# VirtualPlants/tissue_analysis

Measured on AMD Instinct MI355X. Metric: Mvoxels/s full-feature extraction, 1024^3 vol/50k labels; % HBM roofline, higher is better.
Workload: dtype u64; 1 GPU; C4: 1024x1024x1024 uint32, 50000 seeds (21839 labels present), features=0x1f, Z-slab x1; voxels_per_gpu=1073741824, label_dtype=uint32, steps_in_flight=1, per_label_reduce=all

## Files before the change

tissue_analysis_amd/csrc/kernels_basic.hip:

```cpp
#include "ta_kernels.h"

namespace ta {

__global__ void __launch_bounds__(256) init_kernel(uint64_t* sums, int32_t* boxes, uint64_t nlabels,
                                                   uint32_t* flags, uint32_t* cursor, uint64_t* hot_rows) {
    const uint64_t tid = (uint64_t)blockIdx.x * blockDim.x + threadIdx.x;
    const uint64_t nthreads = (uint64_t)gridDim.x * blockDim.x;
    const uint64_t nsum2 = nlabels * NSUM / 2;
    ulonglong2* s2 = reinterpret_cast<ulonglong2*>(sums);
    for (uint64_t i = tid; i < nsum2; i += nthreads) s2[i] = make_ulonglong2(0ull, 0ull);
    const uint64_t nbox2 = nlabels * NBOX / 2;
    int2* b2 = reinterpret_cast<int2*>(boxes);
    for (uint64_t i = tid; i < nbox2; i += nthreads) b2[i] = make_int2(INT32_MAX, INT32_MAX);
    if (tid < NFLAGS) flags[tid] = 0u;
    if (tid == 0) {
        *cursor = 0u;
        *reinterpret_cast<uint64_t**>(flags + HOT_PTR_WORD) = hot_rows;
    }
}

void launch_init_accumulators(hipStream_t s, uint64_t* sums, int32_t* boxes, uint64_t nlabels,
                              uint32_t* flags, uint32_t* pair_cursor, uint64_t* hot_rows) {
    uint64_t work = nlabels * NSUM / 2;
    int blocks = (int)((work + 255) / 256);
// ... 99 lines not shown
        }
    }
    for (uint64_t i = nvec * VEC + tid; i < nvox; i += nthreads) m = max(m, (uint32_t)vol[i]);
#pragma unroll
    for (int off = 32; off > 0; off >>= 1) m = max(m, (uint32_t)__shfl_xor((int)m, off, 64));
    if ((threadIdx.x & 63) == 0) atomicMax(out, m);
}

void launch_max_label(hipStream_t s, const void* vol, int itemsize, uint64_t nvox, uint32_t* out_dev) {
    (void)hipMemsetAsync(out_dev, 0, sizeof(uint32_t), s);
    if (nvox == 0) return;
    uint64_t blocks = (nvox / (16 / itemsize) + 255) / 256;
    if (blocks < 1) blocks = 1;
    if (blocks > 2048) blocks = 2048;
    if (itemsize == 2)
        hipLaunchKernelGGL(max_label_kernel<uint16_t>, dim3((unsigned)blocks), dim3(256), 0, s,
                           (const uint16_t*)vol, nvox, out_dev);
    else
        hipLaunchKernelGGL(max_label_kernel<uint32_t>, dim3((unsigned)blocks), dim3(256), 0, s,
                           (const uint32_t*)vol, nvox, out_dev);
}

constexpr int COLLECT_PER_THREAD = 8;
__device__ __forceinline__ void publish_small(const uint32_t* small, uint32_t* publish, int nwords, int tid) {
    if (tid < nwords) {
        const uint32_t v = __hip_atomic_load(&small[tid], __ATOMIC_RELAXED, __HIP_MEMORY_SCOPE_AGENT);
        __hip_atomic_store(&publish[tid], v, __ATOMIC_RELAXED, __HIP_MEMORY_SCOPE_SYSTEM);
    }
}

__device__ __forceinline__ void pairs_collect_block(const PairTable& pt, uint64_t* out_keys, uint64_t* out_faces,
                                                    uint32_t* cursor, const uint32_t block) {
    __shared__ uint32_t wave_tot[4];
    __shared__ uint32_t block_base;
    const uint64_t cap = (uint64_t)pt.mask + 1;
    const int tid = threadIdx.x, lane = tid & 63, w = tid >> 6;
    const uint64_t lo = (uint64_t)block * (256 * COLLECT_PER_THREAD);
    uint64_t k[COLLECT_PER_THREAD];
    uint32_t mine = 0;
#pragma unroll
    for (int i = 0; i < COLLECT_PER_THREAD; ++i) {
        const uint64_t h = lo + (uint64_t)i * 256 + tid;
        k[i] = h < cap ? pt.keys[h] : EMPTY_KEY;
    }
#pragma unroll
    for (int i = 0; i < COLLECT_PER_THREAD; ++i) mine += k[i] != EMPTY_KEY;
    uint32_t incl = mine;
#pragma unroll
    for (int off = 1; off < 64; off <<= 1) {
        const uint32_t up = (uint32_t)__shfl_up((int)incl, off, 64);
        if (lane >= off) incl += up;
    }
    if (lane == 63) wave_tot[w] = incl;
    __syncthreads();
    if (tid == 0) {
        const uint32_t total = wave_tot[0] + wave_tot[1] + wave_tot[2] + wave_tot[3];
        block_base = total ? atomicAdd(cursor, total) : 0u;
    }
    __syncthreads();
    uint32_t pos = block_base + incl - mine;
    for (int i = 0; i < w; ++i) pos += wave_tot[i];
#pragma unroll
    for (int i = 0; i < COLLECT_PER_THREAD; ++i) {
        if (k[i] == EMPTY_KEY) continue;
        const uint64_t h = lo + (uint64_t)i * 256 + tid;
        out_keys[pos] = k[i];
        out_faces[3ull * pos + 0] = pt.faces[3 * h + 0];
        out_faces[3ull * pos + 1] = pt.faces[3 * h + 1];
        out_faces[3ull * pos + 2] = pt.faces[3 * h + 2];
        ++pos;
        pt.keys[h] = EMPTY_KEY;
        pt.faces[3 * h + 0] = 0; pt.faces[3 * h + 1] = 0; pt.faces[3 * h + 2] = 0;
    }
}

__global__ void __launch_bounds__(256) pairs_collect_kernel(PairTable pt, uint64_t* out_keys,
                                                            uint64_t* out_faces, uint32_t* cursor) {
    pairs_collect_block(pt, out_keys, out_faces, cursor, blockIdx.x);
}

void launch_pairs_collect(hipStream_t s, const PairTable& pt, uint64_t* out_keys, uint64_t* out_faces,
                          uint32_t* cursor) {
    const uint64_t cap = (uint64_t)pt.mask + 1;
    const uint64_t per_block = 256 * COLLECT_PER_THREAD;
    const uint64_t blocks = (cap + per_block - 1) / per_block;
    hipLaunchKernelGGL(pairs_collect_kernel, dim3((unsigned)blocks), dim3(256), 0, s, pt, out_keys,
                       out_faces, cursor);
}

__global__ void __launch_bounds__(256) pairs_insert_kernel(PairTable pt, const uint64_t* keys,
                                                           const uint64_t* faces, uint64_t n,
                                                           uint32_t* flags) {
    for (uint64_t i = (uint64_t)blockIdx.x * blockDim.x + threadIdx.x; i < n;
         i += (uint64_t)gridDim.x * blockDim.x) {
        const uint64_t k = keys[i];
// ... 108 lines not shown
        }
        if (i >= n) continue;
        const uint64_t k = blk[XHDR + i];
        if (k == EMPTY_KEY) continue;
        const uint64_t* f = blk + XHDR + cap + 3 * i;
        pair_add_global(pt, (uint32_t)(k >> 32), (uint32_t)k, f[0], f[1], f[2], flags);
    }
}

void launch_pairs_insert_blocks(hipStream_t s, const PairTable& pt, const uint64_t* blocks, int nblocks,
                                uint64_t cap, uint32_t* flags) {
    const uint64_t total = (uint64_t)nblocks * cap;
    if (total == 0) return;
    uint64_t grid = (total + 255) / 256;
    if (grid > 4096) grid = 4096;
    hipLaunchKernelGGL(pairs_insert_blocks_kernel, dim3((unsigned)grid), dim3(256), 0, s, pt, blocks, nblocks,
                       cap, flags);
}

__global__ void __launch_bounds__(256) pairs_clear_kernel(PairTable pt) {
    const uint64_t cap = (uint64_t)pt.mask + 1;
    for (uint64_t h = (uint64_t)blockIdx.x * blockDim.x + threadIdx.x; h < cap;
         h += (uint64_t)gridDim.x * blockDim.x) {
        pt.keys[h] = EMPTY_KEY;
        pt.faces[3 * h + 0] = 0; pt.faces[3 * h + 1] = 0; pt.faces[3 * h + 2] = 0;
    }
}

void launch_pairs_clear(hipStream_t s, const PairTable& pt) {
    uint64_t cap = (uint64_t)pt.mask + 1;
    uint64_t blocks = (cap + 255) / 256;
    if (blocks > 2048) blocks = 2048;
    hipLaunchKernelGGL(pairs_clear_kernel, dim3((unsigned)blocks), dim3(256), 0, s, pt);
}

struct HotFold {
    const uint64_t* rows; uint32_t nrows;
    const void* vol; int itemsize; int64_t corner;
    uint64_t* sums; int32_t* boxes; uint32_t max_label;
};

__device__ __forceinline__ void hot_reduce_block(const HotFold& H, const uint32_t block, const uint32_t nblocks) {
    __shared__ uint64_t part[256];
    const uint32_t hot = H.itemsize == 2 ? (uint32_t)((const uint16_t*)H.vol)[H.corner] : ((const uint32_t*)H.vol)[H.corner];
    if (hot > H.max_label) return;
    const int col = threadIdx.x & (HOTW - 1), lanegrp = threadIdx.x / HOTW;
    const bool is_sum = col < NSUM;
    int64_t acc = is_sum ? 0 : (int64_t)INT32_MAX;
// ... 394 lines not shown
```

tissue_analysis_amd/csrc/kernels_scan.hip:

```cpp
#include "ta_sweep_common.h"

#include <type_traits>

#include <hip/hip_ext.h>

namespace ta {

constexpr int FCAP = TA_FCAP, RCAP = TA_RCAP;
constexpr uint32_t ROWID_MASK = 0x7FFFFC00u;
constexpr uint32_t ROW_END = 0x80000000u;
constexpr uint32_t NO_ROW = 0xFFFFFFFFu;

typedef __attribute__((address_space(3))) uint32_t* lds_u32;

template <bool ADJ>
struct __attribute__((aligned(16))) ScanWaveLds {
    uint2 frec[ADJ ? FCAP + 1 : 1];
    uint32_t cql[RCAP + 2], cqc[RCAP + 2];
};

template <int NW, bool ADJ, typename PACK>
struct __attribute__((aligned(16))) ScanLds {
    using Pack = PACK;
    ScanWaveLds<ADJ> wave[WAVES];
// ... 124 lines not shown
        k = S.lkeys[h];
    }
    if (slot >= 0) {
        unsigned long long* row = (unsigned long long*)&S.lsum[slot * NW];
        uint64_t w[4];
        LDS::Pack::template pack<MOM2>(L, w);
#ifndef TA_ABL_NOSUMS
#pragma unroll
        for (int k = 0; k < NW; ++k) atomicAdd(row + k, (unsigned long long)w[k]);
#endif
        uint32_t* box = &S.lbox[slot * 8];
        const uint4 cur = *reinterpret_cast<const uint4*>(box);
        const uint2 cur2 = *reinterpret_cast<const uint2*>(box + 4);
#ifdef TA_ABL_NOBOX
        const bool grows = (mna + cur.x + cur2.x == 0x12345u);
#else
        const bool grows = (mna < cur.x) | (mnb < cur.y) | (mnc < cur.z) | (mxa > cur.w) | (mxb > cur2.x) | (mxc > cur2.y);
#endif
        if (grows) {
            atomicMin(box + 0, mna); atomicMin(box + 1, mnb); atomicMin(box + 2, mnc);
            atomicMax(box + 3, mxa); atomicMax(box + 4, mxb); atomicMax(box + 5, mxc);
        }
    } else {
        const SweepArgs* A = cold_args(kp);
        LocalSums Lc;
        Lc.n = L.n; Lc.sa = L.sa; Lc.sb = L.sb; Lc.sc = L.sc; Lc.saa = L.saa; Lc.sab = L.sab;
        Lc.sac = L.sac; Lc.sbb = L.sbb; Lc.sbc = L.sbc; Lc.scc = L.scc;
        uint32_t bx[6];
        bx[0] = mna; bx[1] = mnb; bx[2] = mnc; bx[3] = mxa; bx[4] = mxb; bx[5] = mxc;
        label_spill_global(A->sums, A->boxes, A->flags, A->max_label, label, &Lc, S.frame[0], S.frame[1], S.frame[2], bx);
    }
}

__device__ __forceinline__ uint32_t scan_pair_hash(uint32_t lo, uint32_t hi) {
    const uint32_t h = mad24_const(hi, 0x85EBCBu, mul24_const(lo, 0x9E3779u));
    return (h >> (24 - PSLOTS_LOG2)) & (PSLOTS - 1);
}

template <typename LDS>
__device__ __forceinline__ void scan_pair_add(const SweepArgs* kp, LDS& S, uint32_t lo, uint32_t hi, uint32_t axis, uint32_t h,
                                              uint64_t k) {
    const uint64_t key = ((uint64_t)lo << 32) | hi;
    int slot = -1;
#pragma nounroll
    for (int probe = 0; probe < PPROBE; ++probe) {
        if (k == EMPTY_KEY) {
            k = atomicCAS((unsigned long long*)&S.pkeys[h], (unsigned long long)EMPTY_KEY, (unsigned long long)key);
            if (k == EMPTY_KEY) k = key;
        }
        if (k == key) { slot = (int)h; break; }
        h = (h + 1) & (PSLOTS - 1);
        k = S.pkeys[h];
    }
// ... 256 lines not shown
#ifdef TA_ABL_SHARE1
        unsigned long long* row = (unsigned long long*)&S.lsum[((lslot + (uint32_t)lane) & (LSLOTS - 1)) * NW];
#else
        unsigned long long* row = (unsigned long long*)&S.lsum[lslot * NW];
#endif
        uint64_t w[4];
        LDS::Pack::template pack<MOM2>(L, w);
#pragma unroll
        for (int k = 0; k < NW; ++k) atomicAdd(row + k, (unsigned long long)w[k]);
#ifdef TA_ABL_NOBOXHOT
        const bool grows = false;
#else
        const bool grows = (al < cur.x) | (bl < cur.y) | (c0 < cur.z) | (al > cur.w) | (bl > cur2.x) | (kk - 1u > cur2.y);
#endif
        if (grows) {
            uint32_t* box = &S.lbox[lslot * 8];
            atomicMin(box + 0, al); atomicMin(box + 1, bl); atomicMin(box + 2, c0);
            atomicMax(box + 3, al); atomicMax(box + 4, bl); atomicMax(box + 5, kk - 1u);
        }
    }
    if (spill) {
        if (ppend) { const SweepArgs* A = cold_args(kp); pair_spill_global(A->pairs, A->flags, plo, phi, 2u, 1u); }
        if (lpend) {
            const SweepArgs* A = cold_args(kp);
            LocalSums Lc;
            Lc.n = L.n; Lc.sa = L.sa; Lc.sb = L.sb; Lc.sc = L.sc; Lc.saa = L.saa; Lc.sab = L.sab;
            Lc.sac = L.sac; Lc.sbb = L.sbb; Lc.sbc = L.sbc; Lc.scc = L.scc;
            uint32_t bx[6];
            bx[0] = al; bx[1] = bl; bx[2] = c0; bx[3] = al; bx[4] = bl; bx[5] = kk - 1u;
            label_spill_global(A->sums, A->boxes, A->flags, A->max_label, label, &Lc, S.frame[0], S.frame[1], S.frame[2], bx);
        }
    }
    rcount = rem;
    __builtin_amdgcn_fence(__ATOMIC_ACQ_REL, "wavefront");
}

template <typename T, int VPL>
__device__ __forceinline__ void scan_load_strip(const T* row_c0, bool row_ok, uint32_t lane_off, int64_t c, int64_t n2,
                                                uint32_t (&dst)[VPL], bool& bad) {
    const T* lane_p = reinterpret_cast<const T*>(reinterpret_cast<const char*>(row_c0) + lane_off);
#pragma unroll
    for (int j = 0; j < VPL; ++j) {
        const bool ok = row_ok && c + j < n2;
        dst[j] = ok ? (uint32_t)lane_p[j] : INVALID_LABEL;
        if (sizeof(T) == 4) bad |= ok && dst[j] == INVALID_LABEL;
    }
}

typedef uint32_t u32x4 __attribute__((ext_vector_type(4)));

#define SCAN_VARIANTS(X)                                                             \
    X(scan_kernel,           ROWS_HALO, 104)         \
    X(scan_pad_kernel,       ROWS_HALO, 120)              \
// ... 645 lines not shown
```

tissue_analysis_amd/csrc/ta_api.hip:

```cpp
#include "ta_ctx.h"

#include <cstdarg>
#include <cstdio>
#include <cstdlib>
#include <new>

static thread_local std::string g_err;

int fail(int code, const char* fmt, ...) {
    char buf[512];
    va_list ap;
    va_start(ap, fmt);
    vsnprintf(buf, sizeof(buf), fmt, ap);
    va_end(ap);
    g_err = buf;
    return code;
}

namespace {

int ensure_pair_table(ta_ctx* c, int log2cap) {
    if (c->pair_log2 == log2cap && c->pkeys.p) return TA_OK;
    const uint64_t cap = 1ull << log2cap;
    int rc;
    if ((rc = c->pkeys.reserve(cap * 8)) != TA_OK) return rc;
    if ((rc = c->pfaces.reserve(cap * 24)) != TA_OK) return rc;
    if ((rc = c->out_keys.reserve(cap * 8)) != TA_OK) return rc;
    if ((rc = c->out_faces.reserve(cap * 24)) != TA_OK) return rc;
    c->pair_log2 = log2cap;
    c->table_clean = false;
    return TA_OK;
}

int auto_pair_log2(uint32_t max_label) {
    uint64_t want = 16ull * ((uint64_t)max_label + 1);
    int l = 16;
    while ((1ull << l) < want && l < 28) ++l;
    return l;
}

double sampled_event_density(ta_ctx* c) {
    const int64_t owned = c->mdims[0] - c->first_owned;
    if (owned <= 0 || c->mdims[1] <= 0 || c->mdims[2] <= 0 || !c->vol) return -1.0;
    const int nsample = (int)std::min<int64_t>(8, owned);
    DevBuf d;
    if (d.reserve((uint64_t)nsample * sizeof(uint64_t)) != TA_OK) return -1.0;
    const size_t plane_bytes = (size_t)c->mdims[1] * c->mdims[2] * c->itemsize;
    for (int k = 0; k < nsample; ++k) {
        const int64_t p = c->first_owned + ((2 * k + 1) * owned) / (2 * nsample);
// ... 310 lines not shown
    if (e == hipSuccess && rc == TA_OK) e = hipHostMalloc((void**)&c->h_small, SMALL_WORDS * sizeof(uint32_t), hipHostMallocMapped);
    if (e == hipSuccess && rc == TA_OK) {
        void* dp = nullptr;
        if (hipHostGetDevicePointer(&dp, c->h_small, 0) == hipSuccess) c->h_small_dev = (uint32_t*)dp;
        else (void)hipGetLastError();
    }
    if (e != hipSuccess || rc != TA_OK) {
        if (e != hipSuccess) rc = fail(e == hipErrorOutOfMemory ? TA_ENOMEM : TA_EHIP, "ta_ctx_create: %s", hipGetErrorString(e));
        const std::string keep = g_err;
        (void)ta_ctx_destroy(c);
        g_err = keep;
        return rc;
    }
    memset(c->h_small, 0, SMALL_WORDS * sizeof(uint32_t));
    *out = c;
    return TA_OK;
}

TA_API int ta_ctx_destroy(ta_ctx* c) {
    if (!c) return TA_OK;
    (void)hipSetDevice(c->device);
    if (c->stream) (void)hipStreamSynchronize(c->stream);
    c->owned_vol.release(); c->own_sums.release(); c->own_boxes.release();
    c->pkeys.release(); c->pfaces.release(); c->out_keys.release(); c->out_faces.release();
    c->small.release();
    c->hot_rows.release(); c->sort_buf.release(); c->h_pairs.release();
    c->walls.release(); c->ids.release(); c->shape.release();
    c->sig.release(); c->mesh.release(); c->ov.release(); c->jn.release(); c->wg.release(); c->cc.release(); c->dist.release(); c->near.release(); c->prof.release(); c->sh.release(); c->sm.release(); c->co.release(); c->tp.release(); c->ex.release(); c->rs.release();
    if (c->h_small) (void)hipHostFree(c->h_small);
    destroy_events(c->ev);
    for (auto& e : c->ring) if (e) (void)hipEventDestroy(e);
    if (c->own_stream && c->stream) (void)hipStreamDestroy(c->stream);
    delete c;
    return TA_OK;
}

TA_API int ta_ctx_set_stream(ta_ctx* c, void* hip_stream) {
    if (!c) return fail(TA_EINVAL, "ctx is NULL");
    int rc = use_device(c);
    if (rc != TA_OK) return rc;
    if (c->stream) TA_HIP(hipStreamSynchronize(c->stream));
    if (c->own_stream && c->stream) (void)hipStreamDestroy(c->stream);
    c->stream = nullptr;
    if (hip_stream == TA_STREAM_LEGACY_DEFAULT) {
        c->stream = hipStreamLegacy;
        c->own_stream = false;
    } else if (hip_stream) {
// ... 50 lines not shown
            return fail(TA_EINVAL, "option key %d is read only", key);
        default:
            return fail(TA_EINVAL, "unknown option key %d", key);
    }
}

TA_API int ta_ctx_get_option(ta_ctx* c, int key, int64_t* value) {
    if (!c || !value) return fail(TA_EINVAL, "NULL argument");
    switch (key) {
        case TA_OPT_IMPL: *value = c->impl; return TA_OK;
        case TA_OPT_VOLUME_SLACK: *value = c->volume_slack; return TA_OK;
        case TA_OPT_SWEEP_SHAPE: *value = c->shape.opt; return TA_OK;
        case TA_OPT_SWEEP_SHAPE_USED: *value = c->shape.last; return TA_OK;
        case TA_OPT_TILE_PLANES_USED: *value = c->tile_planes_used; return TA_OK;
        case TA_OPT_TIMING: *value = c->timing; return TA_OK;
        case TA_OPT_TIMING_RING: *value = (int64_t)(c->ring.size() / 2); return TA_OK;
        case TA_OPT_TILE_PLANES: {
            const int shape = c->shape.opt >= 0 ? c->shape.opt : (c->shape.pick >= 0 ? c->shape.pick : 1);
            int planes = c->tile_planes > 0 ? c->tile_planes : ta::sweep_default_tile_planes(c->feature_mask & TA_F_ADJACENCY, c->itemsize, shape);
            if (c->tile_planes <= 0 && c->itemsize == 4 && (c->feature_mask & TA_F_ADJACENCY) && shape == 1 &&
                c->shape.density >= WIDE_SHORTER_TILES_DENSITY && planes > 28) planes = 28;
            *value = planes; return TA_OK;
        }
        case TA_OPT_PAIR_SLOTS: *value = c->pkeys.p ? c->pair_log2 : c->opt_pair_log2; return TA_OK;
        default: return fail(TA_EINVAL, "unknown option key %d", key);
    }
}

TA_API int ta_ctx_synchronize(ta_ctx* c) {
    if (!c) return fail(TA_EINVAL, "ctx is NULL");
    int rc = use_device(c);
    if (rc != TA_OK) return rc;
    TA_HIP(hipStreamSynchronize(c->stream));
    return TA_OK;
}

TA_API int ta_volume_set(ta_ctx* c, const void* host_ptr, int itemsize, const int64_t dims[3],
                  const int64_t strides_bytes[3]) {
    if (!c || !host_ptr || !dims) return fail(TA_EINVAL, "NULL argument");
    if (itemsize != 2 && itemsize != 4) return fail(TA_EINVAL, "itemsize must be 2 (uint16) or 4 (uint32)");
    for (int d = 0; d < 3; ++d)
        if (dims[d] <= 0 || dims[d] > (1ll << 30)) return fail(TA_EINVAL, "dims[%d]=%lld out of range", d, (long long)dims[d]);
    int perm[3] = {0, 1, 2};
    if (strides_bytes) {
        std::stable_sort(perm, perm + 3, [&](int x, int y) {
            const int64_t sx = dims[x] == 1 ? INT64_MAX : strides_bytes[x];
            const int64_t sy = dims[y] == 1 ? INT64_MAX : strides_bytes[y];
// ... 184 lines not shown
    if (feature_mask == 0 || (feature_mask & ~TA_F_ALL)) return fail(TA_EINVAL, "bad feature mask 0x%x", feature_mask);
    if (max_label >= (1u << 28)) return fail(TA_EINVAL, "max_label %u too large for dense per-label rows", max_label);
    int rc = use_device(c);
    if (rc != TA_OK) return rc;
    {
        const long double g0 = (long double)(c->a_origin + c->mdims[0]), nv = (long double)c->mdims[0] * c->mdims[1] * c->mdims[2];
        const long double gm = std::max(g0, std::max((long double)c->mdims[1], (long double)c->mdims[2]));
        if (nv * gm * gm >= 1.8e19L) return fail(TA_EINVAL, "volume too large for exact 64-bit second moments");
    }
    const uint64_t nlabels = (uint64_t)max_label + 1;
    if (c->bound) {
        if (c->bound_max_label != max_label)
            return fail(TA_EINVAL, "bound accumulators are sized for max_label=%u, not %u", c->bound_max_label, max_label);
    } else {
        if ((rc = c->own_sums.reserve(nlabels * ta::NSUM * 8)) != TA_OK) return rc;
        if ((rc = c->own_boxes.reserve(nlabels * ta::NBOX * 4)) != TA_OK) return rc;
        c->sums = (uint64_t*)c->own_sums.p;
        c->boxes = (int32_t*)c->own_boxes.p;
    }
    c->max_label = max_label;
    c->feature_mask = feature_mask;
    {
        const bool adj = feature_mask & TA_F_ADJACENCY;
        int want = c->opt_pair_log2 ? std::max(c->opt_pair_log2, c->pkeys.p ? c->pair_log2 : 0)
                                    : std::max(c->pkeys.p ? c->pair_log2 : 4, adj ? auto_pair_log2(max_label) : 4);
        if ((rc = ensure_pair_table(c, want)) != TA_OK) return rc;
    }
    c->extracted = true;
    c->checked = false;
    c->exchanged = false;
    c->shared_packed = false;
    c->reduced = false;
    c->host_pairs_ready = false;
    return run_extract(c);
}

TA_API int ta_get_labels(ta_ctx* c, uint64_t* count, int32_t* bbox, uint64_t* sum1, uint64_t* sum2) {
    if (!c) return fail(TA_EINVAL, "ctx is NULL");
    int rc = use_device(c);
    if (rc != TA_OK) return rc;
    if ((rc = finish_extract(c)) != TA_OK) return rc;
    const uint64_t n = (uint64_t)c->max_label + 1;
    std::vector<uint64_t> hs;
    std::vector<int32_t> hb;
    try {
        if (count || sum1 || sum2) hs.resize(n * ta::NSUM);
        if (bbox) hb.resize(n * ta::NBOX);
    } catch (...) { return fail(TA_ENOMEM, "out of host memory"); }
// ... 246 lines not shown
```

tissue_analysis_amd/csrc/ta_ctx.h:

```cpp
#pragma once
#include "../../include/tissue_scan.h"
#include "ta_counted.h"
#include "ta_kernels.h"
#include "ta_nearest.h"
#include "ta_parts.h"

#include <algorithm>
#include <cmath>
#include <cstring>
#include <initializer_list>
#include <string>
#include <vector>

int fail(int code, const char* fmt, ...);

#define TA_HIP(expr)                                                                         \
    do {                                                                                     \
        hipError_t e_ = (expr);                                                              \
        if (e_ != hipSuccess)                                                                \
            return fail(e_ == hipErrorOutOfMemory ? TA_ENOMEM : TA_EHIP, "%s: %s (%s:%d)",  \
                        #expr, hipGetErrorString(e_), __FILE__, __LINE__);                   \
    } while (0)

template <bool PINNED> struct Buf {
// ... 282 lines not shown
    int device = 0;
    hipStream_t stream = nullptr;
    bool own_stream = false;
    hipEvent_t ev[4] = {nullptr, nullptr, nullptr, nullptr};
    std::vector<hipEvent_t> ring;
    int timing = 1;
    uint64_t extract_seq = 0, ring_since = 0;

    const void* vol = nullptr;
    DevBuf owned_vol;
    int itemsize = 0;
    int64_t mdims[3] = {0, 0, 0};
    int perm[3] = {0, 1, 2};
    int64_t a_origin = 0;
    int first_owned = 0;

    DevBuf own_sums, own_boxes;
    uint64_t* sums = nullptr;
    int32_t* boxes = nullptr;
    bool bound = false;
    uint32_t bound_max_label = 0;
    uint32_t max_label = 0;

    DevBuf pkeys, pfaces, out_keys, out_faces, small;
    DevBuf hot_rows;
    DevBuf sort_buf;
    int pair_log2 = 0;
    int opt_pair_log2 = 0;
    bool table_clean = false;
    uint32_t* h_small = nullptr;
    uint32_t* h_small_dev = nullptr;

    int impl = 0;
    int tile_planes = 0;
    int tile_planes_used = 0;
    int64_t volume_slack = 0;
    int auto_tile_shift = 0;
    uint64_t last_grid = 0;
    uint32_t feature_mask = 0;
    bool extracted = false, checked = false;
    bool exchanged = false;
    bool shared_packed = false;
    bool reduced = false;
    int64_t npairs = 0;
    PinnedBuf h_pairs;
    bool host_pairs_ready = false;

// ... 127 lines not shown
    return TA_OK;
}
inline int transform_preflight(ta_ctx* c, const char* noun, const double spacing[3], double w[3]) {
    if (!c->vol) return fail(TA_EINVAL, "no label volume set");
    if (c->first_owned != 0 || c->a_origin != 0)
        return fail(TA_EINVAL, "the %s does not take a slab (an exact transform needs halos of unbounded depth)", noun);
    const int rc = extraction_preflight(c, noun);
    if (rc != TA_OK) return rc;
    for (int k = 0; k < 3; ++k) w[k] = spacing[c->perm[k]];
    return TA_OK;
}
inline int check_batch_option(const ta_ctx* c, int64_t columns) {
    if (!c) return fail(TA_EINVAL, "ctx is NULL");
    if (columns < 0 || columns > (1ll << 30)) return fail(TA_EINVAL, "the columns of a batch must be 0 (automatic) or in [1, 2^30]");
    return TA_OK;
}

constexpr int SMALL_WORDS = ta::SMALL_WORDS_DEV;
inline uint32_t* flags_dev(ta_ctx* c) { return (uint32_t*)c->small.p; }
inline uint32_t* cursor_dev(ta_ctx* c) { return (uint32_t*)c->small.p + ta::NFLAGS; }
inline uint32_t* maxlab_dev(ta_ctx* c) { return (uint32_t*)c->small.p + ta::NFLAGS + 1; }
inline ta::PairTable pair_table(ta_ctx* c) {
    ta::PairTable pt;
    pt.keys = (uint64_t*)c->pkeys.p;
    pt.faces = (uint64_t*)c->pfaces.p;
    pt.mask = (uint32_t)((1ull << c->pair_log2) - 1);
    return pt;
}

void walls_on_new_volume(ta_ctx* c);
void sparse_on_new_volume(ta_ctx* c);
void signal_on_new_volume(ta_ctx* c);
void overlap_on_new_volume(ta_ctx* c);
void junctions_on_new_volume(ta_ctx* c);
void wallgeo_on_new_volume(ta_ctx* c);
void components_on_new_volume(ta_ctx* c);
void distance_on_new_volume(ta_ctx* c);
void nearest_on_new_volume(ta_ctx* c);
void profile_on_new_volume(ta_ctx* c);
void profile_on_new_distance(ta_ctx* c);
void profile_on_new_signal(ta_ctx* c);
void sighist_on_new_volume(ta_ctx* c);
void sighist_on_new_signal(ta_ctx* c);
void sigmom_on_new_volume(ta_ctx* c);
void sigmom_on_new_signal(ta_ctx* c);
void cosig_on_new_volume(ta_ctx* c);
void cosig_on_new_signal(ta_ctx* c);
void topology_on_new_volume(ta_ctx* c);
// ... 26 lines not shown
```

tissue_analysis_amd/csrc/ta_device.h:

```cpp
#pragma once
#include <hip/hip_runtime.h>
#include <stdint.h>

#include "ta_range_plan.h"

namespace ta {

constexpr uint32_t INVALID_LABEL = 0xFFFFFFFFu;
constexpr uint64_t EMPTY_KEY = ~0ull;
constexpr int NSUM = 10;
constexpr int NBOX = 6;

enum { FLAG_RANGE = 0, FLAG_PAIR_OVERFLOW = 1, FLAG_LDS_LABEL_SPILL = 2, FLAG_LDS_PAIR_SPILL = 3,
       FLAG_EXCHANGE_OVERFLOW = 4, NFLAGS = 16 };

constexpr int XHDR = 2;
constexpr uint64_t XSTATUS_RANGE = 1, XSTATUS_PAIR_OVERFLOW = 2;

struct DistanceLaunch { uint32_t row_groups = 0, voxel_groups = 0, init_groups = 0, column_launches = 0; };

struct PairTable {
    uint64_t* keys;
    uint64_t* faces;
    uint32_t mask;
};

struct SweepArgs {
    const void* vol;
    int64_t n0, n1, n2;
    int64_t a_origin;
    int32_t first_owned;
    int32_t tile_planes;
    int32_t shape;
    int32_t vec_ok;
    uint32_t max_label;
    uint64_t* sums;
    int32_t* boxes;
    PairTable pairs;
    uint32_t* flags;
};
constexpr int HOTW = 16;
constexpr int HOT_PTR_WORD = NFLAGS + 2;
constexpr int SMALL_WORDS_DEV = NFLAGS + 4;

__device__ __forceinline__ uint32_t hash_u32(uint32_t x) {
    x ^= x >> 16; x *= 0x7feb352du; x ^= x >> 15; x *= 0x846ca68bu; x ^= x >> 16;
    return x;
}
__device__ __forceinline__ uint32_t hash_pair(uint32_t lo, uint32_t hi) {
    return hash_u32(lo * 0x9E3779B1u ^ hash_u32(hi));
}

__device__ __forceinline__ void flush_add(unsigned long long* p, unsigned long long v) { (void)__hip_atomic_fetch_add(p, v, __ATOMIC_RELAXED, __HIP_MEMORY_SCOPE_AGENT); }
__device__ __forceinline__ void flush_min(int32_t* p, int32_t v) { (void)__hip_atomic_fetch_min(p, v, __ATOMIC_RELAXED, __HIP_MEMORY_SCOPE_AGENT); }

__device__ __forceinline__ void pair_add_global_from(const PairTable& pt, uint32_t lo, uint32_t hi, uint64_t f0, uint64_t f1, uint64_t f2,
                                                     uint32_t* flags, uint32_t h, uint64_t k) {
    const uint64_t key = ((uint64_t)lo << 32) | hi;
    for (uint32_t probe = 0; probe < 512u; ++probe) {
        if (k == EMPTY_KEY) {
            k = atomicCAS((unsigned long long*)&pt.keys[h], (unsigned long long)EMPTY_KEY,
                          (unsigned long long)key);
            if (k == EMPTY_KEY) k = key;
        }
        if (k == key) {
            unsigned long long* f = (unsigned long long*)&pt.faces[3ull * h];
            if (f0) flush_add(f + 0, (unsigned long long)f0);
            if (f1) flush_add(f + 1, (unsigned long long)f1);
            if (f2) flush_add(f + 2, (unsigned long long)f2);
            return;
        }
        h = (h + 1) & pt.mask;
        k = __hip_atomic_load(&pt.keys[h], __ATOMIC_RELAXED, __HIP_MEMORY_SCOPE_AGENT);
    }
    atomicOr(&flags[FLAG_PAIR_OVERFLOW], 1u);
}

__device__ inline void pair_add_global(const PairTable& pt, uint32_t lo, uint32_t hi,
                                       uint64_t f0, uint64_t f1, uint64_t f2, uint32_t* flags) {
    const uint64_t key = ((uint64_t)lo << 32) | hi;
    uint32_t h = hash_pair(lo, hi) & pt.mask;
    for (uint32_t probe = 0; probe < 512u; ++probe) {
        uint64_t k = __hip_atomic_load(&pt.keys[h], __ATOMIC_RELAXED, __HIP_MEMORY_SCOPE_AGENT);
        if (k == EMPTY_KEY) {
            k = atomicCAS((unsigned long long*)&pt.keys[h], (unsigned long long)EMPTY_KEY,
                          (unsigned long long)key);
            if (k == EMPTY_KEY) k = key;
        }
        if (k == key) {
            unsigned long long* f = (unsigned long long*)&pt.faces[3ull * h];
            if (f0) atomicAdd(f + 0, (unsigned long long)f0);
            if (f1) atomicAdd(f + 1, (unsigned long long)f1);
            if (f2) atomicAdd(f + 2, (unsigned long long)f2);
            return;
        }
        h = (h + 1) & pt.mask;
    }
    atomicOr(&flags[FLAG_PAIR_OVERFLOW], 1u);
}

template <bool MOM2>
__device__ __forceinline__ void run_moments(uint64_t a0, uint32_t n, uint64_t b, uint64_t c,
                                            uint64_t s[NSUM]) {
    const uint64_t n64 = n;
    const uint64_t t1 = n64 * (n64 - 1) / 2;
    const uint64_t sa = n64 * a0 + t1;
    s[0] = n64; s[1] = sa; s[2] = n64 * b; s[3] = n64 * c;
    if (MOM2) {
        const uint64_t t2 = (n64 - 1) * n64 * (2 * n64 - 1) / 6;
        s[4] = n64 * a0 * a0 + 2 * a0 * t1 + t2;
        s[5] = b * sa; s[6] = c * sa;
        s[7] = n64 * b * b; s[8] = n64 * b * c; s[9] = n64 * c * c;
    } else {
// ... 26 lines not shown
```

tissue_analysis_amd/csrc/ta_sweep_common.h:

```cpp
#pragma once
#include "ta_kernels.h"
#include "ta_sweep_switches.h"

namespace ta {

constexpr int WAVES = TA_WAVES;
constexpr int LSLOTS = TA_LSLOTS;
constexpr int PSLOTS = TA_PSLOTS;
constexpr int ilog2_c(int v) { return v <= 1 ? 0 : 1 + ilog2_c(v >> 1); }
constexpr int LSLOTS_LOG2 = ilog2_c(LSLOTS), PSLOTS_LOG2 = ilog2_c(PSLOTS);
static_assert((1 << LSLOTS_LOG2) == LSLOTS && (1 << PSLOTS_LOG2) == PSLOTS, "table sizes must be powers of two");
constexpr int LPROBE = 16;
constexpr int PPROBE = 32;
constexpr int MAX_TILE_PLANES = 64;
constexpr uint32_t LABEL_LIMIT = 1u << 28;

__device__ __forceinline__ uint32_t lane_shr1(uint32_t src, uint32_t lane0_value) {
    return (uint32_t)__builtin_amdgcn_update_dpp((int)lane0_value, (int)src, 0x138, 0xf, 0xf, false);
}

template <typename T>
__device__ __forceinline__ uint32_t load_uniform_voxel(const T* p) {
    typedef const __attribute__((address_space(4))) uint32_t* cptr;
    const uintptr_t a = reinterpret_cast<uintptr_t>(p);
// ... 37 lines not shown
            L.scc += w[0] & mask(bCC); L.sbc += w[0] >> bCC;
            L.sac += w[1] & mask(bAC); L.saa += w[1] >> bAC;
            L.sc += w[2] & mask(bC); L.sa += (w[2] >> bC) & mask(bA); L.n += w[2] >> (bC + bA);
            L.sab += w[3] & mask(bAB); L.sbb += (w[3] >> bAB) & mask(bBB); L.sb += w[3] >> (bAB + bBB);
        } else {
            L.n += w[0] & 0xffffffffull; L.sb += w[0] >> 32; L.sa += w[1] & 0xffffffffull; L.sc += w[1] >> 32;
        }
    }
};
constexpr int tile_planes_cap(bool adjacency, int itemsize, int vpl) { return adjacency ? (vpl == 4 ? 48 : TA_PLANES_CAP_ADJ8) : (itemsize == 2 ? 32 : 16); }

__device__ __forceinline__ void local_to_global(const LocalSums& L, uint64_t A0, uint64_t B0, uint64_t C0,
                                                uint64_t (&g)[NSUM]) {
    g[0] = L.n;
    g[1] = L.sa + L.n * A0; g[2] = L.sb + L.n * B0; g[3] = L.sc + L.n * C0;
    g[4] = L.saa + 2 * A0 * L.sa + L.n * A0 * A0;
    g[5] = L.sab + A0 * L.sb + B0 * L.sa + L.n * A0 * B0;
    g[6] = L.sac + A0 * L.sc + C0 * L.sa + L.n * A0 * C0;
    g[7] = L.sbb + 2 * B0 * L.sb + L.n * B0 * B0;
    g[8] = L.sbc + B0 * L.sc + C0 * L.sb + L.n * B0 * C0;
    g[9] = L.scc + 2 * C0 * L.sc + L.n * C0 * C0;
}

static __device__ __noinline__ void label_spill_global(uint64_t* sums, int32_t* boxes, uint32_t* flags,
                                                uint32_t max_label, uint32_t label, const LocalSums* L,
                                                uint64_t A0, uint64_t B0, uint64_t C0, const uint32_t* box) {
    atomicAdd(&flags[FLAG_LDS_LABEL_SPILL], 1u);
    if (label > max_label) { atomicOr(&flags[FLAG_RANGE], 1u); return; }
    uint64_t g[NSUM];
    local_to_global(*L, A0, B0, C0, g);
    unsigned long long* row = (unsigned long long*)&sums[(uint64_t)label * NSUM];
    for (int k = 0; k < NSUM; ++k) if (g[k]) atomicAdd(row + k, (unsigned long long)g[k]);
    int32_t* gb = &boxes[(uint64_t)label * NBOX];
    atomicMin(gb + 0, (int32_t)(A0 + box[0])); atomicMin(gb + 3, -(int32_t)(A0 + box[3]));
    atomicMin(gb + 1, (int32_t)(B0 + box[1])); atomicMin(gb + 4, -(int32_t)(B0 + box[4]));
    atomicMin(gb + 2, (int32_t)(C0 + box[2])); atomicMin(gb + 5, -(int32_t)(C0 + box[5]));
}

static __device__ __noinline__ void pair_spill_global(PairTable pt, uint32_t* flags, uint32_t lo, uint32_t hi,
                                               uint32_t axis, uint32_t count) {
    atomicAdd(&flags[FLAG_LDS_PAIR_SPILL], 1u);
    pair_add_global(pt, lo, hi, axis == 0 ? count : 0, axis == 1 ? count : 0, axis == 2 ? count : 0, flags);
}

__device__ __forceinline__ uint64_t range_sum1(uint64_t x0, uint64_t n) { return n * x0 + n * (n - 1) / 2; }
__device__ __forceinline__ uint64_t range_sum2(uint64_t x0, uint64_t n) {
    return n * x0 * x0 + x0 * n * (n - 1) + (n - 1) * n * (2 * n - 1) / 6;
}

template <typename T>
__device__ __forceinline__ uint32_t hot_label_of(const SweepArgs& A) {
    return load_uniform_voxel<T>(reinterpret_cast<const T*>(A.vol) + (int64_t)A.first_owned * A.n1 * A.n2);
}
__device__ __forceinline__ uint64_t* hot_rows_of(const SweepArgs& A) {
    typedef uint64_t* const __attribute__((address_space(4)))* cpp;
    return *reinterpret_cast<cpp>(reinterpret_cast<uintptr_t>(A.flags + HOT_PTR_WORD));
}
__device__ __forceinline__ void hot_row_init(const SweepArgs& A, const int tid, const uint32_t wg) {
    uint64_t* rows = hot_rows_of(A);
// ... 35 lines not shown
            base = (uint32_t)__builtin_amdgcn_readfirstlane((int)base);
            if (live) plist[base + __builtin_amdgcn_mbcnt_hi((uint32_t)(m >> 32), __builtin_amdgcn_mbcnt_lo((uint32_t)m, 0u))] = (uint16_t)i;
        }
    }
    __syncthreads();
    const int nl = (int)S.fcnt[0], np = ADJ ? (int)S.fcnt[1] : 0;

    constexpr int NS = MOM2 ? NSUM : 4;
    static_assert(!ADJ || (PSLOTS <= 2 * NT && (size_t)LSLOTS * NSUM * 8 <= sizeof(S.pkeys) + sizeof(S.pcnt)),
                  "the flush takes two pairs a thread and stages the labels' sums where the pair table was");
    if constexpr (ADJ) {
        static_assert(offsetof(LDS, pcnt) == offsetof(LDS, pkeys) + sizeof(S.pkeys), "the staged sums run from the pair keys on into the pair counts");
        uint64_t pkey[2], gkey[2]; uint32_t pf[2][3], ghome[2]; bool plive[2];
#pragma unroll
        for (int q = 0; q < 2; ++q) {
            const int j = NT - 1 - tid + q * NT;
            plive[q] = j < np;
            pkey[q] = gkey[q] = 0ull; ghome[q] = 0u; pf[q][0] = pf[q][1] = pf[q][2] = 0u;
#ifndef TA_ABL_NOFLUSH_PAIRS
            if (plive[q]) {
                const int i = plist[j];
                pkey[q] = S.pkeys[i];
                ghome[q] = hash_pair((uint32_t)(pkey[q] >> 32), (uint32_t)pkey[q]) & A.pairs.mask;
                gkey[q] = __hip_atomic_load(&A.pairs.keys[ghome[q]], __ATOMIC_RELAXED, __HIP_MEMORY_SCOPE_AGENT);
                pf[q][0] = S.pcnt[i * 3 + 0]; pf[q][1] = S.pcnt[i * 3 + 1]; pf[q][2] = S.pcnt[i * 3 + 2];
            }
#endif
        }
        __syncthreads();
        uint64_t* const stage = reinterpret_cast<uint64_t*>(&S.pkeys[0]);
        uint64_t* const hot_rows = HOT ? hot_rows_of(A) : nullptr;
        uint64_t* const hr = hot_rows + (uint64_t)wg * HOTW;
#ifndef TA_ABL_NOFLUSH_LABELS
        for (int j = tid; j < nl; j += NT) {
            const int i = llist[j];
            const uint32_t label = S.lkeys[i];
            LocalSums L;
            L.n = L.sa = L.sb = L.sc = L.saa = L.sab = L.sac = L.sbb = L.sbc = L.scc = 0;
            for (int pass = 0; pass < 1; ++pass) {
                uint64_t w[4] = {0ull, 0ull, 0ull, 0ull};
#pragma unroll
                for (int k = 0; k < NW; ++k) w[k] = S.lsum[i * NW + k];
                LDS::Pack::template unpack_add<MOM2>(w, L);
            }
            uint64_t g[NSUM];
            local_to_global(L, A0, B0, C0, g);
            const bool ok = label <= A.max_label;
// ... 74 lines not shown
```

Measured before the change: 1.110 million Mvoxels/s.

## Interleave pair-table keys and face counts into 32-byte slots

Replaces the separate key and face arrays of the global pair hash table with an array-of-structs where each 32-byte slot holds the key and its three face counts, so a probe hit and its atomic adds touch one sector instead of two distant lines. The collect and clear kernels now move whole slots. Separately, the cold label-spill path now takes scalar sums and packed 8-bit box coordinates instead of a local struct and array, which is meant to avoid scratch stack traffic in the noinline call. Risks: linear probing now strides 32 bytes per probe instead of 8, so long probe chains touch more cache lines, and the packed box assumes tile-local coordinates fit in 8 bits.

```diff
diff --git a/tissue_analysis_amd/csrc/kernels_basic.hip b/tissue_analysis_amd/csrc/kernels_basic.hip
--- a/tissue_analysis_amd/csrc/kernels_basic.hip
+++ b/tissue_analysis_amd/csrc/kernels_basic.hip
@@ -145,6 +145,7 @@
 }
 
 constexpr int COLLECT_PER_THREAD = 8;
+constexpr PairSlot FREE_SLOT = {EMPTY_KEY, {0ull, 0ull, 0ull}};
 __device__ __forceinline__ void publish_small(const uint32_t* small, uint32_t* publish, int nwords, int tid) {
     if (tid < nwords) {
         const uint32_t v = __hip_atomic_load(&small[tid], __ATOMIC_RELAXED, __HIP_MEMORY_SCOPE_AGENT);
@@ -159,15 +160,15 @@
     const uint64_t cap = (uint64_t)pt.mask + 1;
     const int tid = threadIdx.x, lane = tid & 63, w = tid >> 6;
     const uint64_t lo = (uint64_t)block * (256 * COLLECT_PER_THREAD);
-    uint64_t k[COLLECT_PER_THREAD];
+    PairSlot s[COLLECT_PER_THREAD];
     uint32_t mine = 0;
 #pragma unroll
     for (int i = 0; i < COLLECT_PER_THREAD; ++i) {
         const uint64_t h = lo + (uint64_t)i * 256 + tid;
-        k[i] = h < cap ? pt.keys[h] : EMPTY_KEY;
-    }
-#pragma unroll
-    for (int i = 0; i < COLLECT_PER_THREAD; ++i) mine += k[i] != EMPTY_KEY;
+        s[i] = h < cap ? pt.slots[h] : FREE_SLOT;
+    }
+#pragma unroll
+    for (int i = 0; i < COLLECT_PER_THREAD; ++i) mine += s[i].key != EMPTY_KEY;
     uint32_t incl = mine;
 #pragma unroll
     for (int off = 1; off < 64; off <<= 1) {
@@ -185,15 +186,14 @@
     for (int i = 0; i < w; ++i) pos += wave_tot[i];
 #pragma unroll
     for (int i = 0; i < COLLECT_PER_THREAD; ++i) {
-        if (k[i] == EMPTY_KEY) continue;
+        if (s[i].key == EMPTY_KEY) continue;
         const uint64_t h = lo + (uint64_t)i * 256 + tid;
-        out_keys[pos] = k[i];
-        out_faces[3ull * pos + 0] = pt.faces[3 * h + 0];
-        out_faces[3ull * pos + 1] = pt.faces[3 * h + 1];
-        out_faces[3ull * pos + 2] = pt.faces[3 * h + 2];
+        out_keys[pos] = s[i].key;
+        out_faces[3ull * pos + 0] = s[i].f[0];
+        out_faces[3ull * pos + 1] = s[i].f[1];
+        out_faces[3ull * pos + 2] = s[i].f[2];
         ++pos;
-        pt.keys[h] = EMPTY_KEY;
-        pt.faces[3 * h + 0] = 0; pt.faces[3 * h + 1] = 0; pt.faces[3 * h + 2] = 0;
+        pt.slots[h] = FREE_SLOT;
     }
 }
 
@@ -348,8 +348,7 @@
     const uint64_t cap = (uint64_t)pt.mask + 1;
     for (uint64_t h = (uint64_t)blockIdx.x * blockDim.x + threadIdx.x; h < cap;
          h += (uint64_t)gridDim.x * blockDim.x) {
-        pt.keys[h] = EMPTY_KEY;
-        pt.faces[3 * h + 0] = 0; pt.faces[3 * h + 1] = 0; pt.faces[3 * h + 2] = 0;
+        pt.slots[h] = FREE_SLOT;
     }
 }
 
diff --git a/tissue_analysis_amd/csrc/kernels_scan.hip b/tissue_analysis_amd/csrc/kernels_scan.hip
--- a/tissue_analysis_amd/csrc/kernels_scan.hip
+++ b/tissue_analysis_amd/csrc/kernels_scan.hip
@@ -170,13 +170,8 @@
             atomicMax(box + 3, mxa); atomicMax(box + 4, mxb); atomicMax(box + 5, mxc);
         }
     } else {
-        const SweepArgs* A = cold_args(kp);
-        LocalSums Lc;
-        Lc.n = L.n; Lc.sa = L.sa; Lc.sb = L.sb; Lc.sc = L.sc; Lc.saa = L.saa; Lc.sab = L.sab;
-        Lc.sac = L.sac; Lc.sbb = L.sbb; Lc.sbc = L.sbc; Lc.scc = L.scc;
-        uint32_t bx[6];
-        bx[0] = mna; bx[1] = mnb; bx[2] = mnc; bx[3] = mxa; bx[4] = mxb; bx[5] = mxc;
-        label_spill_global(A->sums, A->boxes, A->flags, A->max_label, label, &Lc, S.frame[0], S.frame[1], S.frame[2], bx);
+        label_spill_global(cold_args(kp), label, L.n, L.sa, L.sb, L.sc, L.saa, L.sab, L.sac, L.sbb, L.sbc, L.scc,
+                           S.frame[0], S.frame[1], S.frame[2], pack_box3(mna, mnb, mnc), pack_box3(mxa, mxb, mxc));
     }
 }
 
@@ -479,13 +474,8 @@
     if (spill) {
         if (ppend) { const SweepArgs* A = cold_args(kp); pair_spill_global(A->pairs, A->flags, plo, phi, 2u, 1u); }
         if (lpend) {
-            const SweepArgs* A = cold_args(kp);
-            LocalSums Lc;
-            Lc.n = L.n; Lc.sa = L.sa; Lc.sb = L.sb; Lc.sc = L.sc; Lc.saa = L.saa; Lc.sab = L.sab;
-            Lc.sac = L.sac; Lc.sbb = L.sbb; Lc.sbc = L.sbc; Lc.scc = L.scc;
-            uint32_t bx[6];
-            bx[0] = al; bx[1] = bl; bx[2] = c0; bx[3] = al; bx[4] = bl; bx[5] = kk - 1u;
-            label_spill_global(A->sums, A->boxes, A->flags, A->max_label, label, &Lc, S.frame[0], S.frame[1], S.frame[2], bx);
+            label_spill_global(cold_args(kp), label, L.n, L.sa, L.sb, L.sc, L.saa, L.sab, L.sac, L.sbb, L.sbc, L.scc,
+                               S.frame[0], S.frame[1], S.frame[2], pack_box3(al, bl, c0), pack_box3(al, bl, kk - 1u));
         }
     }
     rcount = rem;
diff --git a/tissue_analysis_amd/csrc/ta_api.hip b/tissue_analysis_amd/csrc/ta_api.hip
--- a/tissue_analysis_amd/csrc/ta_api.hip
+++ b/tissue_analysis_amd/csrc/ta_api.hip
@@ -20,11 +20,10 @@
 namespace {
 
 int ensure_pair_table(ta_ctx* c, int log2cap) {
-    if (c->pair_log2 == log2cap && c->pkeys.p) return TA_OK;
+    if (c->pair_log2 == log2cap && c->pslots.p) return TA_OK;
     const uint64_t cap = 1ull << log2cap;
     int rc;
-    if ((rc = c->pkeys.reserve(cap * 8)) != TA_OK) return rc;
-    if ((rc = c->pfaces.reserve(cap * 24)) != TA_OK) return rc;
+    if ((rc = c->pslots.reserve(cap * sizeof(ta::PairSlot))) != TA_OK) return rc;
     if ((rc = c->out_keys.reserve(cap * 8)) != TA_OK) return rc;
     if ((rc = c->out_faces.reserve(cap * 24)) != TA_OK) return rc;
     c->pair_log2 = log2cap;
@@ -381,7 +380,7 @@
     (void)hipSetDevice(c->device);
     if (c->stream) (void)hipStreamSynchronize(c->stream);
     c->owned_vol.release(); c->own_sums.release(); c->own_boxes.release();
-    c->pkeys.release(); c->pfaces.release(); c->out_keys.release(); c->out_faces.release();
+    c->pslots.release(); c->out_keys.release(); c->out_faces.release();
     c->small.release();
     c->hot_rows.release(); c->sort_buf.release(); c->h_pairs.release();
     c->walls.release(); c->ids.release(); c->shape.release();
@@ -478,7 +477,7 @@
                 c->shape.density >= WIDE_SHORTER_TILES_DENSITY && planes > 28) planes = 28;
             *value = planes; return TA_OK;
         }
-        case TA_OPT_PAIR_SLOTS: *value = c->pkeys.p ? c->pair_log2 : c->opt_pair_log2; return TA_OK;
+        case TA_OPT_PAIR_SLOTS: *value = c->pslots.p ? c->pair_log2 : c->opt_pair_log2; return TA_OK;
         default: return fail(TA_EINVAL, "unknown option key %d", key);
     }
 }
@@ -709,8 +708,8 @@
     c->feature_mask = feature_mask;
     {
         const bool adj = feature_mask & TA_F_ADJACENCY;
-        int want = c->opt_pair_log2 ? std::max(c->opt_pair_log2, c->pkeys.p ? c->pair_log2 : 0)
-                                    : std::max(c->pkeys.p ? c->pair_log2 : 4, adj ? auto_pair_log2(max_label) : 4);
+        int want = c->opt_pair_log2 ? std::max(c->opt_pair_log2, c->pslots.p ? c->pair_log2 : 0)
+                                    : std::max(c->pslots.p ? c->pair_log2 : 4, adj ? auto_pair_log2(max_label) : 4);
         if ((rc = ensure_pair_table(c, want)) != TA_OK) return rc;
     }
     c->extracted = true;
diff --git a/tissue_analysis_amd/csrc/ta_ctx.h b/tissue_analysis_amd/csrc/ta_ctx.h
--- a/tissue_analysis_amd/csrc/ta_ctx.h
+++ b/tissue_analysis_amd/csrc/ta_ctx.h
@@ -328,7 +328,7 @@
     uint32_t bound_max_label = 0;
     uint32_t max_label = 0;
 
-    DevBuf pkeys, pfaces, out_keys, out_faces, small;
+    DevBuf pslots, out_keys, out_faces, small;
     DevBuf hot_rows;
     DevBuf sort_buf;
     int pair_log2 = 0;
@@ -502,8 +502,8 @@
 inline uint32_t* maxlab_dev(ta_ctx* c) { return (uint32_t*)c->small.p + ta::NFLAGS + 1; }
 inline ta::PairTable pair_table(ta_ctx* c) {
     ta::PairTable pt;
-    pt.keys = (uint64_t*)c->pkeys.p;
-    pt.faces = (uint64_t*)c->pfaces.p;
+    pt.slots = (ta::PairSlot*)c->pslots.p;
+    pt.unused = 0;
     pt.mask = (uint32_t)((1ull << c->pair_log2) - 1);
     return pt;
 }
diff --git a/tissue_analysis_amd/csrc/ta_device.h b/tissue_analysis_amd/csrc/ta_device.h
--- a/tissue_analysis_amd/csrc/ta_device.h
+++ b/tissue_analysis_amd/csrc/ta_device.h
@@ -19,9 +19,11 @@
 
 struct DistanceLaunch { uint32_t row_groups = 0, voxel_groups = 0, init_groups = 0, column_launches = 0; };
 
+struct alignas(32) PairSlot { uint64_t key; uint64_t f[3]; };
+static_assert(sizeof(PairSlot) == 32, "a slot is one 32-byte sector");
 struct PairTable {
-    uint64_t* keys;
-    uint64_t* faces;
+    PairSlot* slots;
+    uint64_t unused;
     uint32_t mask;
 };
 
@@ -59,19 +61,19 @@
     const uint64_t key = ((uint64_t)lo << 32) | hi;
     for (uint32_t probe = 0; probe < 512u; ++probe) {
         if (k == EMPTY_KEY) {
-            k = atomicCAS((unsigned long long*)&pt.keys[h], (unsigned long long)EMPTY_KEY,
+            k = atomicCAS((unsigned long long*)&pt.slots[h].key, (unsigned long long)EMPTY_KEY,
                           (unsigned long long)key);
             if (k == EMPTY_KEY) k = key;
         }
         if (k == key) {
-            unsigned long long* f = (unsigned long long*)&pt.faces[3ull * h];
+            unsigned long long* f = (unsigned long long*)pt.slots[h].f;
             if (f0) flush_add(f + 0, (unsigned long long)f0);
             if (f1) flush_add(f + 1, (unsigned long long)f1);
             if (f2) flush_add(f + 2, (unsigned long long)f2);
             return;
         }
         h = (h + 1) & pt.mask;
-        k = __hip_atomic_load(&pt.keys[h], __ATOMIC_RELAXED, __HIP_MEMORY_SCOPE_AGENT);
+        k = __hip_atomic_load(&pt.slots[h].key, __ATOMIC_RELAXED, __HIP_MEMORY_SCOPE_AGENT);
     }
     atomicOr(&flags[FLAG_PAIR_OVERFLOW], 1u);
 }
@@ -81,14 +83,14 @@
     const uint64_t key = ((uint64_t)lo << 32) | hi;
     uint32_t h = hash_pair(lo, hi) & pt.mask;
     for (uint32_t probe = 0; probe < 512u; ++probe) {
-        uint64_t k = __hip_atomic_load(&pt.keys[h], __ATOMIC_RELAXED, __HIP_MEMORY_SCOPE_AGENT);
+        uint64_t k = __hip_atomic_load(&pt.slots[h].key, __ATOMIC_RELAXED, __HIP_MEMORY_SCOPE_AGENT);
         if (k == EMPTY_KEY) {
-            k = atomicCAS((unsigned long long*)&pt.keys[h], (unsigned long long)EMPTY_KEY,
+            k = atomicCAS((unsigned long long*)&pt.slots[h].key, (unsigned long long)EMPTY_KEY,
                           (unsigned long long)key);
             if (k == EMPTY_KEY) k = key;
         }
         if (k == key) {
-            unsigned long long* f = (unsigned long long*)&pt.faces[3ull * h];
+            unsigned long long* f = (unsigned long long*)pt.slots[h].f;
             if (f0) atomicAdd(f + 0, (unsigned long long)f0);
             if (f1) atomicAdd(f + 1, (unsigned long long)f1);
             if (f2) atomicAdd(f + 2, (unsigned long long)f2);
diff --git a/tissue_analysis_amd/csrc/ta_sweep_common.h b/tissue_analysis_amd/csrc/ta_sweep_common.h
--- a/tissue_analysis_amd/csrc/ta_sweep_common.h
+++ b/tissue_analysis_amd/csrc/ta_sweep_common.h
@@ -83,19 +83,23 @@
     g[9] = L.scc + 2 * C0 * L.sc + L.n * C0 * C0;
 }
 
-static __device__ __noinline__ void label_spill_global(uint64_t* sums, int32_t* boxes, uint32_t* flags,
-                                                uint32_t max_label, uint32_t label, const LocalSums* L,
-                                                uint64_t A0, uint64_t B0, uint64_t C0, const uint32_t* box) {
+__device__ __forceinline__ uint32_t pack_box3(uint32_t a, uint32_t b, uint32_t c) { return a | (b << 8) | (c << 16); }
+static __device__ __noinline__ void label_spill_global(const SweepArgs* A, uint32_t label, uint64_t n, uint64_t sa, uint64_t sb, uint64_t sc,
+                                                uint64_t saa, uint64_t sab, uint64_t sac, uint64_t sbb, uint64_t sbc, uint64_t scc,
+                                                uint32_t A0, uint32_t B0, uint32_t C0, uint32_t mins, uint32_t maxs) {
+    uint32_t* const flags = A->flags;
     atomicAdd(&flags[FLAG_LDS_LABEL_SPILL], 1u);
-    if (label > max_label) { atomicOr(&flags[FLAG_RANGE], 1u); return; }
+    if (label > A->max_label) { atomicOr(&flags[FLAG_RANGE], 1u); return; }
+    const LocalSums L = {n, sa, sb, sc, saa, sab, sac, sbb, sbc, scc};
     uint64_t g[NSUM];
-    local_to_global(*L, A0, B0, C0, g);
-    unsigned long long* row = (unsigned long long*)&sums[(uint64_t)label * NSUM];
+    local_to_global(L, A0, B0, C0, g);
+    unsigned long long* row = (unsigned long long*)&A->sums[(uint64_t)label * NSUM];
+#pragma unroll
     for (int k = 0; k < NSUM; ++k) if (g[k]) atomicAdd(row + k, (unsigned long long)g[k]);
-    int32_t* gb = &boxes[(uint64_t)label * NBOX];
-    atomicMin(gb + 0, (int32_t)(A0 + box[0])); atomicMin(gb + 3, -(int32_t)(A0 + box[3]));
-    atomicMin(gb + 1, (int32_t)(B0 + box[1])); atomicMin(gb + 4, -(int32_t)(B0 + box[4]));
-    atomicMin(gb + 2, (int32_t)(C0 + box[2])); atomicMin(gb + 5, -(int32_t)(C0 + box[5]));
+    int32_t* gb = &A->boxes[(uint64_t)label * NBOX];
+    atomicMin(gb + 0, (int32_t)(A0 + (mins & 255u)));         atomicMin(gb + 3, -(int32_t)(A0 + (maxs & 255u)));
+    atomicMin(gb + 1, (int32_t)(B0 + ((mins >> 8) & 255u)));  atomicMin(gb + 4, -(int32_t)(B0 + ((maxs >> 8) & 255u)));
+    atomicMin(gb + 2, (int32_t)(C0 + (mins >> 16)));          atomicMin(gb + 5, -(int32_t)(C0 + (maxs >> 16)));
 }
 
 static __device__ __noinline__ void pair_spill_global(PairTable pt, uint32_t* flags, uint32_t lo, uint32_t hi,
@@ -177,7 +181,7 @@
                 const int i = plist[j];
                 pkey[q] = S.pkeys[i];
                 ghome[q] = hash_pair((uint32_t)(pkey[q] >> 32), (uint32_t)pkey[q]) & A.pairs.mask;
-                gkey[q] = __hip_atomic_load(&A.pairs.keys[ghome[q]], __ATOMIC_RELAXED, __HIP_MEMORY_SCOPE_AGENT);
+                gkey[q] = __hip_atomic_load(&A.pairs.slots[ghome[q]].key, __ATOMIC_RELAXED, __HIP_MEMORY_SCOPE_AGENT);
                 pf[q][0] = S.pcnt[i * 3 + 0]; pf[q][1] = S.pcnt[i * 3 + 1]; pf[q][2] = S.pcnt[i * 3 + 2];
             }
 #endif
```

Result: faster. 1.173 million Mvoxels/s (median of 6 runs) (+5.7%).
